# TheShadow29/VidSitu

Hardware: AMD Instinct MI355X
Metric: clips/s (10s@32x224x224) SlowFast+TxEnc fwd+bwd (higher is better)
Workload: dtype bf16

## Files before the change

### include/vidsitu_hip.h

```cpp
#ifndef VIDSITU_HIP_H
#define VIDSITU_HIP_H

#include <stddef.h>
#include <stdint.h>

#ifdef __cplusplus
extern "C" {
#endif

typedef enum vs_status {
  VS_OK = 0,
  VS_ERR_BAD_ARG = -1,
  VS_ERR_UNSUPPORTED = -2,
  VS_ERR_WORKSPACE = -3,
  VS_ERR_LAUNCH = -4
} vs_status;

#define VS_CONV_AFFINE 1
#define VS_CONV_RESIDUAL 2
#define VS_CONV_RELU 4
#define VS_CONV_STATS 8
#define VS_CONV_NAIVE 16
#define VS_CONV_TILE(id) (((id) + 1) << 8)
#define VS_CONV_RING(ns) (((ns) & 7) << 16)
// ... 40 lines not shown
int vs_stem_conv_wgrad(const void* dy, const void* x4, float* dwp, int N, int T, int H, int W,
                       int Cout, int kT, int dy_ld, void* workspace, size_t ws_bytes, void* stream);

int vs_conv_fwd(const void* x, const void* w, void* y, const vs_conv_desc* d, const float* scale,
                const float* shift, const void* residual, float* stats_partial,
                void* workspace, size_t ws_bytes, void* stream);
int vs_conv_stats_rows(const vs_conv_desc* d);
size_t vs_conv_workspace_bytes(const vs_conv_desc* d, int dgrad);
int vs_conv_plan(const vs_conv_desc* d, int dgrad, int* out);
int vs_conv_fwd_bc_fusable(const vs_conv_desc* d, int cout_c);
int vs_conv_fwd_bc(const void* x, const void* w_b, const vs_conv_desc* d, const float* scale_b,
                   const float* shift_b, const void* w_c, int cout_c, const float* scale_c,
                   const float* shift_c, const void* residual, int res_ld, void* y, int y_ld, int relu_c,
                   void* stream);

int vs_conv_dgrad(const void* dy, const void* wt, void* dx, const vs_conv_desc* d,
                  const void* residual, void* workspace, size_t ws_bytes, void* stream);

int vs_conv_dgrad_bnstats_rows(const vs_conv_desc* d);
int vs_conv_dgrad_bnstats(const void* dy, const void* wt, void* dx, const vs_conv_desc* d, const void* residual,
                          const void* bn_y, int bn_y_ld, const uint8_t* relu_bits, const float* mean,
                          const float* invstd, const float* gamma, const float* beta, float* stats_partial,
                          void* workspace, size_t ws_bytes, void* stream);

typedef struct vs_dgrad_epilogue {
  const void* residual;
  const uint8_t* residual_bits;
  const void* bn_y;
  int bn_y_ld;
  const uint8_t* relu_bits;
  const float* mean;
  const float* invstd;
  const float* gamma;
  const float* beta;
  float* stats_partial;
  const void* bn_y2;
  int bn_y2_ld;
  const float* mean2;
  const float* invstd2;
  float* stats_partial2;
} vs_dgrad_epilogue;
int vs_conv_dgrad_ex(const void* dy, const void* wt, void* dx, const vs_conv_desc* d,
                     const vs_dgrad_epilogue* ep, void* workspace, size_t ws_bytes, void* stream);
int vs_weight_transpose(const void* w, void* wt, int Cout, int taps, int Cin, void* stream);
int vs_weight_transpose_batched(const void* src, void* dst, const int64_t* table, int n,
                                int64_t total, void* stream);
int vs_transpose_f32_batched(const float* src, float* dst, const int64_t* table, int n, int64_t total,
                             void* stream);
int vs_weight_transpose_tiled(const void* src, void* dst, const int64_t* table, const int64_t* tile_first,
                              int n, int64_t total_tiles, int elem_bytes, void* stream);

#define VS_WGRAD_NODEEP (1 << 12)
#define VS_WGRAD_FORCEDEEP (1 << 13)
size_t vs_conv_wgrad_workspace_bytes(const vs_conv_desc* d);
int vs_conv_wgrad(const void* dy, const void* x, float* dw, const vs_conv_desc* d,
                  void* workspace, size_t ws_bytes, void* stream);
typedef struct vs_wgrad_item {
  const void* dy;
  const void* x;
  float* dw;
  vs_conv_desc d;
} vs_wgrad_item;
int vs_conv_wgrad_group_ok(const vs_wgrad_item* items, int n);
size_t vs_conv_wgrad_group_workspace_bytes(const vs_wgrad_item* items, int n);
int vs_conv_wgrad_group(const vs_wgrad_item* items, int n, void* workspace, size_t ws_bytes, void* stream);
int vs_conv_wgrad_partial(const void* dy, const void* x, float* dw, const vs_conv_desc* d, void* slabs,
                          size_t slab_bytes, int* splits, void* stream);
int64_t vs_wgrad_reduce_blocks(int64_t elements);
int vs_wgrad_reduce(const float* slabs, float* dw, int64_t elements, int splits, void* stream);
int vs_wgrad_reduce_batched(const int64_t* table, int n_entries, int64_t total_blocks, void* stream);
int vs_wgrad_reduce_defer(int mode);
int vs_wgrad_reduce_flush(void);

int vs_bn_finalize(const float* partials, int nparts, double count, const float* gamma,
                   const float* beta, float* running_mean, float* running_var, float momentum,
                   float eps, float* scale, float* shift, float* mean, float* invstd, int C,
                   void* stream);
size_t vs_bn_finalize_workspace_bytes(void);
int vs_bn_finalize_ws(const float* partials, int nparts, double count, const float* gamma, const float* beta,
                      float* running_mean, float* running_var, float momentum, float eps, float* scale,
                      float* shift, float* mean, float* invstd, int C, void* workspace, size_t ws_bytes,
                      void* stream);
int vs_bn_partials_reduce(const float* partials, int nparts, float* out, int C, int G,
                          void* stream);
int vs_bn_apply(const void* y, const float* scale, const float* shift, const void* residual,
                void* out, int64_t rows, int C, int y_ld, int res_ld, int out_ld, int relu,
                void* stream);
int vs_bn_apply_mask(const void* y, const float* scale, const float* shift, const void* residual,
                     void* out, uint8_t* relu_bits, int64_t rows, int C, int y_ld, int res_ld,
                     int out_ld, void* stream);
int vs_bn_apply2(const void* y, const float* scale, const float* shift, const void* y2, const float* scale2,
                 const float* shift2, void* out, uint8_t* relu_bits, int64_t rows, int C, int y_ld, int y2_ld,
                 int out_ld, void* stream);
int vs_bn_bwd_reduce(const void* dz, const void* z, const void* y, const float* mean,
                     const float* invstd, const float* gamma, const float* beta, float* partial,
                     int64_t rows, int C, int dz_ld, int z_ld, int y_ld, int relu, void* stream);
int vs_bn_bwd_reduce_rows(int64_t rows, int C);
int vs_bn_bwd_finalize(const float* partial, int nparts, float* dgamma, float* dbeta, int C,
                       void* stream);
int vs_bn_bwd_finalize_ws(const float* partial, int nparts, float* dgamma, float* dbeta, int C, void* workspace,
                          size_t ws_bytes, void* stream);
int vs_bn_bwd_apply(const void* dz, const void* z, const void* y, const float* mean,
                    const float* invstd, const float* gamma, const float* beta,
                    const float* dgamma, const float* dbeta, void* dy, void* dres, int64_t rows,
                    int C, int dz_ld, int z_ld, int y_ld, int dy_ld, int dres_ld, int relu,
                    void* stream);
// ... 211 lines not shown
```

### vidsitu_amd/_lib.py

```python
import ctypes as C
import os
import subprocess

_HERE = os.path.dirname(os.path.abspath(__file__))
LIB_PATH = os.environ.get("VS_LIB_PATH") or os.path.join(_HERE, "libvidsitu_hip.so")
CSRC_DIR = os.path.join(_HERE, "csrc")

VS_CONV_AFFINE = 1
VS_CONV_RESIDUAL = 2
VS_CONV_RELU = 4
VS_CONV_STATS = 8
VS_CONV_NAIVE = 16
VS_CONV_SPLITK = 1 << 15
VS_CONV_NOCLASS = 1 << 19
VS_CONV_NOHALO = 1 << 21
VS_CONV_FORCEHALO = 1 << 22
VS_CONV_NOPW = 1 << 23
VS_CONV_FORCEPW = 1 << 24
VS_CONV_DIRECTBNB = 1 << 25
VS_CONV_BNB2 = 1 << 26
VS_CONV_NODEEP = 1 << 27
VS_CONV_FORCEDEEP = 1 << 28
VS_CONV_SPLITK_IL = 1 << 29
VS_CONV_NOSPLITK_IL = 1 << 30
VS_WGRAD_NODEEP = 1 << 12
VS_WGRAD_FORCEDEEP = 1 << 13


def VS_CONV_TILE(tile_id):
    return (tile_id + 1) << 8


def VS_CONV_RING(stages):
    return (stages & 7) << 16


class ConvDesc(C.Structure):

    _fields_ = [
        (n, C.c_int32)
        for n in (
            "N Ti Hi Wi Cin To Ho Wo Cout kT kH kW sT sH sW pT pH pW x_ld y_ld res_ld flags"
        ).split()
    ]


class DgradEpilogue(C.Structure):

    _fields_ = [("residual", C.c_void_p), ("residual_bits", C.c_void_p), ("bn_y", C.c_void_p),
                ("bn_y_ld", C.c_int32), ("relu_bits", C.c_void_p), ("mean", C.c_void_p),
                ("invstd", C.c_void_p), ("gamma", C.c_void_p), ("beta", C.c_void_p),
                ("stats_partial", C.c_void_p), ("bn_y2", C.c_void_p), ("bn_y2_ld", C.c_int32),
                ("mean2", C.c_void_p), ("invstd2", C.c_void_p), ("stats_partial2", C.c_void_p)]


class WgradItem(C.Structure):

    _fields_ = [("dy", C.c_void_p), ("x", C.c_void_p), ("dw", C.c_void_p), ("d", ConvDesc)]


_p, _i, _i64, _f, _d, _sz = C.c_void_p, C.c_int, C.c_int64, C.c_float, C.c_double, C.c_size_t
_u32, _u64 = C.c_uint32, C.c_uint64
_dp = C.POINTER(ConvDesc)

SIGNATURES = {
    "vs_last_error_string": (C.c_char_p, []),
    "vs_version": (_i, []),
    "vs_launch_count": (_i64, []),
    "vs_pack_input": (_i, [_p, _i, _p, _i, _i, _i, _i, _i, _i, _p]),
    "vs_frames_u8_pack": (_i, [_p, _p, _p, _i, _i, _i, _i, _i, _i, _p, _p, _i, _p]),
    "vs_stem_conv_fwd": (_i, [_p, _p, _p, _i, _i, _i, _i, _i, _i, _i, _i, _p, _p, _p, _p]),
    "vs_stem_stats_rows": (_i, [_i, _i, _i, _i]),
    "vs_stem_wgrad_workspace_bytes": (_sz, [_i, _i, _i, _i, _i, _i]),
    "vs_stem_conv_wgrad": (_i, [_p, _p, _p, _i, _i, _i, _i, _i, _i, _i, _p, _sz, _p]),
    "vs_conv_fwd": (_i, [_p, _p, _p, _dp, _p, _p, _p, _p, _p, _sz, _p]),
    "vs_conv_stats_rows": (_i, [_dp]),
    "vs_conv_workspace_bytes": (_sz, [_dp, _i]),
    "vs_conv_plan": (_i, [_dp, _i, _p]),
    "vs_conv_fwd_bc_fusable": (_i, [_dp, _i]),
# ... 185 lines not shown
```

### vidsitu_amd/csrc/conv_wgrad.hip

```cpp
#include <stdlib.h>

#include "common.h"

#include <mutex>
#include <type_traits>
#include "glue_bodies.h"

typedef __attribute__((ext_vector_type(4))) short s16x4;
typedef __attribute__((address_space(3))) s16x4 lds_s16x4;

struct WgradP {
  const uint16_t* dy;
  const uint16_t* x;
  float* out;
  int P;
  int Cout, Kp, Cin, x_ld, dy_ld;
  int To, Ho, Wo, Ti, Hi, Wi;
  int kT, kH, kW, sT, sH, sW, pT, pH, pW;
  int tilesM, tilesN, S, rows_per_split;
  unsigned x_bytes, dy_bytes;
  int xcd_order;
  int dbg;
};

#define WG_OOB 0x80000000u

#define WG_ROWTAB 1024

__device__ __forceinline__ int wg_swz_chunk(int row) {
  return ((row & 3) << 1) | (((row >> 3) & 1) << 3);
}

#ifndef WG_NARROW_DEPTH
#define WG_NARROW_DEPTH 3
#endif
constexpr int wg_depth(int bm) { return bm <= 32 ? WG_NARROW_DEPTH : 2; }

template <int BM, int BN, int WM, int WN, int MODE>
__global__ __launch_bounds__(256) void conv_wgrad_kernel(WgradP p) {
  extern __shared__ __attribute__((aligned(16))) char smem[];
  constexpr int D = wg_depth(BM), R = D - 1;
  static_assert(D >= 2 && R * 64 < WG_ROWTAB / 2, "loads never run past the table half being rebuilt");
  constexpr int TM = BM / WM, TN = BN / WN;
  constexpr int MR = TM / 16, NR = TN / 16;
  constexpr int CM = BM / 8, CN = BN / 8;
  constexpr int RPM = 256 / CM, RPN = 256 / CN;
  constexpr int IM = (64 + RPM - 1) / RPM, IN = (64 + RPN - 1) / RPN;
  constexpr int IMG = 64 * 256;
  constexpr int STAGE = 2 * IMG;
  static_assert(WM * WN == 4, "4 waves");

  const int tid = threadIdx.x;
  int bid = blockIdx.x;
  if (p.xcd_order) {
    const int nwg = gridDim.x, q = nwg >> 3, r = nwg & 7, xcd = blockIdx.x & 7;
    bid = (xcd < r ? xcd * (q + 1) : r * (q + 1) + (xcd - r) * q) + (blockIdx.x >> 3);
  }
  const int ntile = p.tilesM * p.tilesN;
  const int s = bid / ntile;
// ... 843 lines not shown
      for (int u = 0; u < 8; ++u) v[u] = *(const float4*)(slabs + (long long)(s + u) * n + i * 4);
#pragma unroll
      for (int u = 0; u < 8; ++u) {
        acc.x += v[u].x;
        acc.y += v[u].y;
        acc.z += v[u].z;
        acc.w += v[u].w;
      }
    }
    for (; s < s1; ++s) {
      const float4 v = *(const float4*)(slabs + (long long)s * n + i * 4);
      acc.x += v.x;
      acc.y += v.y;
      acc.z += v.z;
      acc.w += v.w;
    }
  }
  part[sl][col] = acc;
  __syncthreads();
  if (sl == 0 && i < n4) {
    float4 t = part[0][col];
    for (int k = 1; k < 16; ++k) {
      const float4 v = part[k][col];
      t.x += v.x;
      t.y += v.y;
      t.z += v.z;
      t.w += v.w;
    }
    *(float4*)(dw + i * 4) = t;
  }
}

extern "C" int vs_wgrad_reduce_batched(const int64_t* table, int n_entries, int64_t total_blocks, void* stream) {
  VS_CHECK_ARG(table && n_entries > 0 && total_blocks > 0, "bad args");
  hipLaunchKernelGGL(wgrad_reduce_batched_kernel, dim3((unsigned)total_blocks), dim3(256), 0, (hipStream_t)stream,
                     (const long long*)table, n_entries);
  VS_CHECK_LAUNCH();
  return VS_OK;
}

extern "C" int64_t vs_wgrad_reduce_blocks(int64_t n) { return (n / 4 + 15) / 16; }

extern "C" int vs_wgrad_reduce(const float* slabs, float* dw, int64_t n, int splits, void* stream) {
  VS_CHECK_ARG(slabs && dw && n > 0 && splits > 1, "bad args");
  hipLaunchKernelGGL(wgrad_reduce_kernel, dim3((unsigned)wgrad_reduce_vblocks(n, splits)), dim3(256), 0, (hipStream_t)stream,
                     slabs, dw, (long long)n, splits);
  VS_CHECK_LAUNCH();
  return VS_OK;
}

struct WgCfg {
  int bm, bn, S, rows_per_split, tilesM, tilesN;
  int deep;
};


static bool wg_deep_plan(const vs_conv_desc* d, WgCfg* c) {
  static const int mode = [] { const char* e = getenv("VS_WGRAD_DEEP"); return e ? atoi(e) : 1; }();
  const bool force = mode == 2 || (d->flags & VS_WGRAD_FORCEDEEP);
  if (mode == 0 || (d->flags & VS_WGRAD_NODEEP)) return false;
  if (((d->flags >> 8) & 0xf) || ((d->flags >> 16) & 7) || ((d->flags >> 24) & 0xff)) return false;
  const int taps = d->kT * d->kH * d->kW;
  const int Kp = taps * d->Cin;
  const long long P = (long long)d->N * d->To * d->Ho * d->Wo;
  if (taps > 31 || Kp % 8 != 0 || d->Cout % 8 != 0) return false;
  const int tilesM = (d->Cout + 127) / 128, tilesN = (Kp + 255) / 256;
  const long long tiles = (long long)tilesM * tilesN;
  const double row_eff = (double)d->Cout / (128.0 * tilesM), col_eff = (double)Kp / (256.0 * tilesN);
  long long S = 256 / tiles;
  const long long maxS = P / 512;
  if (S > maxS) S = maxS;
  const long long slab_cap = (64ll << 20) / ((long long)d->Cout * Kp * 4);
  if (S > slab_cap) S = slab_cap;
  if (S < 1) S = 1;
  long long rps = (P + S - 1) / S;
  rps = (rps + 31) / 32 * 32;
  S = (P + rps - 1) / rps;
  if (!force && (row_eff < 0.9 || col_eff < 0.75 || tiles * S < 128 || tiles > 256 || rps < 512)) return false;
  static const long long min_p = [] { const char* e = getenv("VS_WGRAD_DEEP_MINP"); return e ? atoll(e) : 3000ll; }();
  if (!force && P < min_p) return false;
  if (tiles * S > 65535) return false;
  c->bm = 128;
  c->bn = 256;
  c->tilesM = tilesM;
  c->tilesN = tilesN;
  c->S = (int)S;
  c->rows_per_split = (int)rps;
  c->deep = 1;
  return true;
}

static const int kWgTiles[8][2] = {{128, 128}, {128, 64}, {64, 128}, {64, 64}, {32, 128}, {32, 64}, {16, 128}, {16, 64}};

static WgCfg wg_pick(const vs_conv_desc* d) {
  WgCfg c;
  c.deep = 0;
  if (wg_deep_plan(d, &c)) return c;
  const int Kp = d->kT * d->kH * d->kW * d->Cin;
  const long long P = (long long)d->N * d->To * d->Ho * d->Wo;
  c.bm = d->Cout >= 128 ? 128 : (d->Cout >= 64 ? 64 : (d->Cout >= 32 ? 32 : 16));
  c.bn = Kp >= 128 ? 128 : 64;
  if (d->Cout <= 16) c.bn = Kp > 64 ? 128 : 64;
  else if (d->Cout <= 32) c.bn = 64;
  const int forced = (d->flags >> 8) & 0xf;
  if (forced >= 1 && forced <= 8) {
    c.bm = kWgTiles[forced - 1][0];
    c.bn = kWgTiles[forced - 1][1];
  }
  c.tilesM = (d->Cout + c.bm - 1) / c.bm;
  c.tilesN = (Kp + c.bn - 1) / c.bn;
  const long long tiles = (long long)c.tilesM * c.tilesN;
  static const long long slots = [] {
    const char* e = getenv("VS_WGRAD_SLOTS");
    return e ? atoll(e) : 384ll;
  }();
  static const long long small_slots = [] {
    const char* e = getenv("VS_WGRAD_SLOTS_SMALL");
    return e ? atoll(e) : 512ll;
  }();
  long long target = (d->Cout <= 32) ? small_slots : slots;
  const int forced_slots = (d->flags >> 24) & 0xff;
  if (forced_slots) target = 8ll * forced_slots;
  long long S = target / tiles;
  static const long long s1_tiles = [] {
    const char* e = getenv("VS_WGRAD_S1_TILES");
    return e ? atoll(e) : 128ll;
  }();
  if (s1_tiles > 0 && tiles >= s1_tiles && !forced_slots) S = 1;
  const long long maxS = (P + 511) / 512;
  if (S > maxS) S = maxS;
  const long long slab_cap = (64ll << 20) / ((long long)d->Cout * Kp * 4);
  if (S > slab_cap) S = slab_cap;
  if (S > 1024) S = 1024;
  if (S < 1) S = 1;
  long long rps = (P + S - 1) / S;
  rps = (rps + 63) / 64 * 64;
  S = (P + rps - 1) / rps;
  c.S = (int)S;
  c.rows_per_split = (int)rps;
  return c;
}

extern "C" size_t vs_conv_wgrad_workspace_bytes(const vs_conv_desc* d) {
  const WgCfg c = wg_pick(d);
  if (c.S <= 1) return 0;
  return (size_t)c.S * d->Cout * d->kT * d->kH * d->kW * d->Cin * sizeof(float);
}

static bool pair_take_wgrad(const WgradP& p, int grid, size_t smem, int mode, hipStream_t st);
// ... 270 lines not shown
        while (t0 < nt) {
          const long long chunk = pos >> 5;
          const int room = 32 - (int)(pos & 31), c = nt - t0 < room ? nt - t0 : room;
          const int x = (int)(chunk & 7), slot0 = (int)(chunk >> 3) * 32 + (int)(pos & 31);
          if (cnt[x] == WGG_JOBS || slot0 + c > 510) { fits = false; break; }
          g.jobtab[x][cnt[x]++] = ((unsigned)slot0 << 23) | ((unsigned)a << 18) | ((unsigned)sp << 12) | (unsigned)t0;
          t0 += c;
          pos += c;
        }
      }
    }
    if (fits) {
      const long long chunks = (pos + 31) >> 5;
      int mx = 0;
      for (int x = 0; x < 8; ++x) {
        long long sl = 0;
        for (long long c = x; c < chunks; c += 8) sl = (c >> 3) * 32 + ((c == chunks - 1 && (pos & 31)) ? (pos & 31) : 32);
        g.jobend[x] = (unsigned short)sl;
        if ((int)sl > mx) mx = (int)sl;
      }
#ifdef VS_WGG_DEBUG
      for (int x = 0; x < 8; ++x) {
        fprintf(stderr, "xcd %d (%d slots):", x, (int)g.jobend[x]);
        for (int i = 0; i < cnt[x]; ++i) fprintf(stderr, " [slot %u p %u s %u t %u]", g.jobtab[x][i] >> 23, (g.jobtab[x][i] >> 18) & 31, (g.jobtab[x][i] >> 12) & 63, g.jobtab[x][i] & 4095);
        fprintf(stderr, "\n");
      }
      for (int a = 0; a < n; ++a) fprintf(stderr, "problem %d: tiles %d x %d S %d rps %d count %d\n", a, g.p[a].tilesM, g.p[a].tilesN, g.p[a].S, g.p[a].rows_per_split, g.count[a]);
#endif
      g.jobs = 1;
      grid = 8 * mx;
    }
  }
  static std::once_flag gattr;
  std::call_once(gattr, [] {
    (void)hipFuncSetAttribute((const void*)conv_wgrad_deep_group_kernel, hipFuncAttributeMaxDynamicSharedMemorySize, 160 * 1024);
  });
  const size_t smem = (size_t)WGD_NU * WGD_UNIT + 2 * WGD_TAB * sizeof(int2);
  hipLaunchKernelGGL(conv_wgrad_deep_group_kernel, dim3(grid), dim3(512), smem, (hipStream_t)stream, g);
  VS_CHECK_LAUNCH();
  if (r.n > 0) {
    hipLaunchKernelGGL(wgrad_reduce_group_kernel, dim3((unsigned)r.first[r.n]), dim3(256), 0, (hipStream_t)stream, r);
    VS_CHECK_LAUNCH();
  }
  return VS_OK;
}

static int wgrad_impl(const void* dy, const void* x, float* dw, const vs_conv_desc* d, void* workspace,
                      size_t ws_bytes, void* stream, bool reduce_now, int* splits_out) {
  VS_CHECK_ARG(d && dy && x && dw, "null argument");
  VS_CHECK_ARG(d->Cin % 8 == 0 && d->Cout % 8 == 0, "Cin and Cout must be multiples of 8");
  VS_CHECK_ARG(d->x_ld % 8 == 0 && d->y_ld % 8 == 0, "row pitches must be multiples of 8");
  VS_CHECK_ARG((long long)d->N * d->Ti * d->Hi * d->Wi < (1ll << 31), "too many positions");
  const WgCfg c = wg_pick(d);
  const size_t need = vs_conv_wgrad_workspace_bytes(d);
  if (need > 0 && (workspace == nullptr || ws_bytes < need)) {
    vs_set_error("vs_conv_wgrad: workspace too small (%zu < %zu)", ws_bytes, need);
    return VS_ERR_WORKSPACE;
  }
  if (g_pending.have && ((const void*)g_pending.r.slabs == workspace || g_pending.r.dw == dw)) pending_flush();
  WgradP p;
  {
    const int rc = wg_fill_params(p, dy, x, c.S > 1 ? (float*)workspace : dw, d, c);
    if (rc) return rc;
  }
  {
    static const int xo = [] { const char* e = getenv("VS_WGRAD_XCD"); return e ? atoi(e) : 1; }();
    p.xcd_order = xo && (c.tilesM * c.tilesN <= 32 || xo == 2 || (c.S % 8 == 0 && c.tilesM * c.tilesN <= 64));
    static const int dbg = [] { const char* e = getenv("VS_WGRAD_DBG"); return e ? atoi(e) : 0; }();
    p.dbg = dbg;
  }
  p.rows_per_split = c.rows_per_split;
  const bool dense = (d->kT * d->kH * d->kW == 1) && d->sT == 1 && d->sH == 1 && d->sW == 1 &&
                     d->pT == 0 && d->pH == 0 && d->pW == 0;
  const int mode = dense ? 0 : 1;
  hipStream_t st = (hipStream_t)stream;
  const int fring = (d->flags >> 16) & 7;
  int ring = fring == 1 ? 0 : (fring >= 2 ? (fring > 3 ? 3 : fring) : (c.bm == 128 ? 2 : 0));
  if (d->kT * d->kH * d->kW > 31) ring = 0;
  int rc;
  if (c.deep) {
    static std::once_flag dattr;
    std::call_once(dattr, [] {
      (void)hipFuncSetAttribute((const void*)conv_wgrad_deep_kernel<0, false>, hipFuncAttributeMaxDynamicSharedMemorySize, 160 * 1024);
      (void)hipFuncSetAttribute((const void*)conv_wgrad_deep_kernel<1, false>, hipFuncAttributeMaxDynamicSharedMemorySize, 160 * 1024);
      (void)hipFuncSetAttribute((const void*)conv_wgrad_deep_kernel<0, true>, hipFuncAttributeMaxDynamicSharedMemorySize, 160 * 1024);
      (void)hipFuncSetAttribute((const void*)conv_wgrad_deep_kernel<1, true>, hipFuncAttributeMaxDynamicSharedMemorySize, 160 * 1024);
    });
    static const int stag = [] { const char* e = getenv("VS_WGRAD_DEEP_STAG"); return e ? atoi(e) : 1; }();
    const size_t smem = (size_t)WGD_NU * WGD_UNIT + 2 * WGD_TAB * sizeof(int2);
    const int grid = p.tilesM * p.tilesN * p.S;
    if (stag && mode == 0) hipLaunchKernelGGL((conv_wgrad_deep_kernel<0, true>), dim3(grid), dim3(512), smem, st, p);
    else if (stag) hipLaunchKernelGGL((conv_wgrad_deep_kernel<1, true>), dim3(grid), dim3(512), smem, st, p);
    else if (mode == 0) hipLaunchKernelGGL((conv_wgrad_deep_kernel<0, false>), dim3(grid), dim3(512), smem, st, p);
    else hipLaunchKernelGGL((conv_wgrad_deep_kernel<1, false>), dim3(grid), dim3(512), smem, st, p);
    VS_CHECK_LAUNCH();
    rc = VS_OK;
  } else if (c.bm == 128 && c.bn == 128) rc = wg_launch<128, 128, 2, 2>(p, mode, ring, st);
  else if (c.bm == 128) rc = wg_launch<128, 64, 2, 2>(p, mode, ring, st);
  else if (c.bm == 64 && c.bn == 128) rc = wg_launch<64, 128, 2, 2>(p, mode, ring, st);
  else if (c.bm == 64) rc = wg_launch<64, 64, 2, 2>(p, mode, ring, st);
  else if (c.bm == 32 && c.bn == 128) rc = wg_launch<32, 128, 1, 4>(p, mode, ring, st);
  else if (c.bm == 32) rc = wg_launch<32, 64, 1, 4>(p, mode, ring, st);
  else if (c.bn == 128) rc = wg_launch<16, 128, 1, 4>(p, mode, ring, st);
  else rc = wg_launch<16, 64, 1, 4>(p, mode, ring, st);
  if (rc) return rc;
  if (splits_out) *splits_out = c.S;
  if (c.S > 1 && reduce_now) {
    const long long n = (long long)d->Cout * p.Kp;
    const long long grid = wgrad_reduce_vblocks(n, c.S);
    if (!pair_defer_reduce((const float*)workspace, dw, n, c.S) &&
        !pending_stash((const float*)workspace, dw, n, c.S, st)) {
      hipLaunchKernelGGL(wgrad_reduce_kernel, dim3((unsigned)grid), dim3(256), 0, st,
                         (const float*)workspace, dw, n, c.S);
      VS_CHECK_LAUNCH();
    }
  }
  return VS_OK;
}

extern "C" int vs_conv_wgrad(const void* dy, const void* x, float* dw, const vs_conv_desc* d,
                             void* workspace,
                             size_t ws_bytes, void* stream) {
  return wgrad_impl(dy, x, dw, d, workspace, ws_bytes, stream, true, nullptr);
}

extern "C" int vs_conv_wgrad_partial(const void* dy, const void* x, float* dw, const vs_conv_desc* d, void* slabs,
                                     size_t slab_bytes, int* splits, void* stream) {
  VS_CHECK_ARG(splits != nullptr, "null splits");
  return wgrad_impl(dy, x, dw, d, slabs, slab_bytes, stream, false, splits);
}
```

### vidsitu_amd/ops.py

```python
import ctypes as C

import torch

from . import _lib
from ._lib import (
    VS_CONV_AFFINE,
    VS_CONV_BNB2,
    VS_CONV_DIRECTBNB,
    VS_CONV_FORCEDEEP,
    VS_CONV_FORCEHALO,
    VS_CONV_FORCEPW,
    VS_CONV_NAIVE,
    VS_CONV_NOCLASS,
    VS_CONV_NODEEP,
    VS_CONV_NOHALO,
    VS_CONV_NOPW,
    VS_CONV_NOSPLITK_IL,
    VS_CONV_RELU,
    VS_CONV_RESIDUAL,
    VS_CONV_RING,
    VS_CONV_SPLITK,
    VS_CONV_SPLITK_IL,
    VS_CONV_STATS,
    VS_CONV_TILE,
    VS_WGRAD_FORCEDEEP,
    VS_WGRAD_NODEEP,
    ConvDesc,
)

BF16 = torch.bfloat16


def _stream():
    return C.c_void_p(torch.cuda.current_stream().cuda_stream)


def _ptr(t):
    if t is None:
        return None
    if not t.is_cuda:
        raise _lib.VsError("HIP op called with a non-GPU tensor (no CPU fallback exists)")
    return C.c_void_p(t.data_ptr())


def new_act(n, c, t, h, w, device, ctot=None, c_off=0, dtype=BF16, zero=False):
    ctot = c if ctot is None else ctot
    alloc = torch.zeros if zero else torch.empty
    buf = alloc((n, t, h, w, ctot), dtype=dtype, device=device)
    return buf.permute(0, 4, 1, 2, 3)[:, c_off : c_off + c]


def channel_slice(x, c_off, c):
    return x[:, c_off : c_off + c]


def act_ld(x):
    n, c, t, h, w = x.shape
    s = x.stride()
    ld = s[4] if w > 1 else (s[3] if h > 1 else (s[2] if t > 1 else s[0]))
    ok = (c == 1 or s[1] == 1) and ld >= c
    ok = ok and (w == 1 or s[4] == ld) and (h == 1 or s[3] == w * ld)
    ok = ok and (t == 1 or s[2] == h * w * ld) and (n == 1 or s[0] == t * h * w * ld)
    if not ok or x.dtype != BF16:
        raise _lib.VsError(f"not a bf16 channels-last activation: shape {tuple(x.shape)} stride {s}")
    if ld % 8 or (x.storage_offset() % 8):
        raise _lib.VsError("activation pitch / channel offset must be multiples of 8")
    return ld


def act_rows(x):
    n, c, t, h, w = x.shape
    return n * t * h * w


def pack_input(x, cpad=8):
    x = x.contiguous()
    n, c, t, h, w = x.shape
    y = new_act(n, cpad, t, h, w, x.device)
    _lib.call(
# ... 354 lines not shown
        return out

    def flush(self):
        if not self.pending:
            return
        sig = tuple(self.pending)
        ent = self.tables.get(sig)
        if ent is None:
            rows, first = [], 0
            lib = _lib.load()
            for slab_ptr, dw_ptr, n, S in self.pending:
                rows.append([slab_ptr, dw_ptr, n, S, first])
                first += int(lib.vs_wgrad_reduce_blocks(n))
            dev = torch.device("cuda", torch.cuda.current_device())
            ent = self.tables[sig] = (torch.tensor(rows, dtype=torch.int64, device=dev), len(rows), first)
        table, n_ent, blocks = ent
        _lib.call("vs_wgrad_reduce_batched", _ptr(table), n_ent, blocks, _stream())
        self.pending = []


WG_TILES = [(128, 128), (128, 64), (64, 128), (64, 64), (32, 128), (32, 64), (16, 128), (16, 64)]


WGRAD_GROUP_MAX = 20


def _wgrad_items(items):
    arr = (_lib.WgradItem * len(items))()
    for i, (dy, x, k, s, p, out) in enumerate(items):
        if not out.permute(0, 2, 3, 4, 1).is_contiguous() or out.dtype != torch.float32:
            raise _lib.VsError("conv_wgrad out must be fp32 with [Cout][taps][Cin] memory")
        arr[i].dy, arr[i].x, arr[i].dw = dy.data_ptr(), x.data_ptr(), out.data_ptr()
        arr[i].d = make_desc(x.shape, act_ld(x), dy.shape, act_ld(dy), k, s, p, 0)
        _ptr(dy), _ptr(x), _ptr(out)
    return arr


def conv_wgrad_group_ok(items):
    if not 1 <= len(items) <= WGRAD_GROUP_MAX:
        return False
    return bool(_lib.load().vs_conv_wgrad_group_ok(_wgrad_items(items), len(items)))


def conv_wgrad_group(items):
    if _WHATIF_WGRAD:
        return
    arr = _wgrad_items(items)
    need = int(_lib.load().vs_conv_wgrad_group_workspace_bytes(arr, len(items)))
    ws = _workspace(need, items[0][0].device, "wgrad") if need else None
    _lib.call("vs_conv_wgrad_group", arr, len(items), _ptr(ws), C.c_size_t(ws.numel() if ws is not None else 0),
              _stream())


def conv_wgrad(dy, x, k, s, p, out=None, ring=0, batch=None, tile=None, slots=0, deep=True):
    cout, cin = dy.shape[1], x.shape[1]
    if out is None:
        out = torch.empty((cout, *k, cin), dtype=torch.float32, device=x.device).permute(0, 4, 1, 2, 3)
    elif not out.permute(0, 2, 3, 4, 1).is_contiguous() or out.dtype != torch.float32:
        raise _lib.VsError("conv_wgrad out must be fp32 with [Cout][taps][Cin] memory")
    if batch is not None:
        return batch.wgrad(dy, x, k, s, p, out, ring)
    if _WHATIF_WGRAD:
        return out
    flags = ((ring & 7) << 16) | (((tile + 1) << 8) if tile is not None else 0) | (((slots // 8) & 0xff) << 24)
    if not deep:
        flags |= VS_WGRAD_NODEEP
    elif deep == "force":
        flags |= VS_WGRAD_FORCEDEEP
    d = make_desc(x.shape, act_ld(x), dy.shape, act_ld(dy), k, s, p, flags)
    need = _lib.load().vs_conv_wgrad_workspace_bytes(C.byref(d))
    ws = _workspace(need, x.device, "wgrad") if need else None
    _lib.call("vs_conv_wgrad", _ptr(dy), _ptr(x), _ptr(out), C.byref(d), _ptr(ws),
              C.c_size_t(ws.numel() if ws is not None else 0), _stream())
    return out


import os as _os
_WHATIF = int(_os.environ.get("VS_WHATIF", "0"))
_BN_TWO_LEVEL = int(_os.environ.get("VS_BN_TWO_LEVEL", "512"))
BN_FIN2 = _os.environ.get("VS_BN_FIN2", "1") != "0"
_fin_ws = [0]
_whatif_const = {}


def _fin_ws_bytes():
    if not _fin_ws[0]:
        _fin_ws[0] = int(_lib.load().vs_bn_finalize_workspace_bytes())
    return _fin_ws[0]



def bn_finalize(partials, count, gamma, beta, running_mean, running_var, momentum, eps, train):
    c = gamma.numel()
    dev = gamma.device
    scale = torch.empty(c, dtype=torch.float32, device=dev)
    shift = torch.empty(c, dtype=torch.float32, device=dev)
    mean = torch.empty(c, dtype=torch.float32, device=dev)
    invstd = torch.empty(c, dtype=torch.float32, device=dev)
    nparts = partials.shape[0] if train else 0
    if train and _WHATIF & 1:
        k = (c, str(dev))
        if k not in _whatif_const:
            _whatif_const[k] = (torch.ones(c, device=dev), torch.zeros(c, device=dev), torch.zeros(c, device=dev),
                                torch.ones(c, device=dev))
        return _whatif_const[k]
    if train and BN_FIN2:
        ws = _workspace(_fin_ws_bytes(), dev, "fin")
        _lib.call("vs_bn_finalize_ws", _ptr(partials), nparts, float(count), _ptr(gamma), _ptr(beta),
                  _ptr(running_mean), _ptr(running_var), float(momentum), float(eps), _ptr(scale), _ptr(shift),
                  _ptr(mean), _ptr(invstd), c, _ptr(ws), C.c_size_t(ws.numel()), _stream())
        return scale, shift, mean, invstd
    if train and nparts > _BN_TWO_LEVEL:
        lvl1 = torch.empty((32, 2, c), dtype=torch.float32, device=dev)
        _lib.call("vs_bn_partials_reduce", _ptr(partials), nparts, _ptr(lvl1), c, 32, _stream())
        partials, nparts = lvl1, 32
    _lib.call("vs_bn_finalize", _ptr(partials) if train else None, nparts, float(count),
              _ptr(gamma), _ptr(beta), _ptr(running_mean), _ptr(running_var), float(momentum),
              float(eps), _ptr(scale), _ptr(shift), _ptr(mean), _ptr(invstd), c, _stream())
    return scale, shift, mean, invstd


# ... 956 lines not shown
```

Measured before the change: 742.5.

## Add patch-tiled wgrad kernel for small-channel 1x3x3 convolutions

Adds a dedicated weight-gradient kernel for stride-1, padding-1 1x3x3 convolutions with up to 64 channels. Each block DMAs spatial patches of x, with halo, and of dy into LDS through a 2- or 3-deep buffer ring. It builds all nine taps from the shared patch using transposed LDS reads and MFMA, and writes per-split slabs that the existing reduction sums. By default it is used only for the 8→8 and 64→64 shapes of the SlowFast bottlenecks, and only when there are enough positions. The goal is to stop re-reading im2col-style data for each tap. The cost is extra plan and launch complexity and a workspace size that is now computed from the patch plan.

```diff
diff --git a/include/vidsitu_hip.h b/include/vidsitu_hip.h
--- a/include/vidsitu_hip.h
+++ b/include/vidsitu_hip.h
@@ -116,6 +116,8 @@
 
 #define VS_WGRAD_NODEEP (1 << 12)
 #define VS_WGRAD_FORCEDEEP (1 << 13)
+#define VS_WGRAD_NOPATCH (1 << 14)
+#define VS_WGRAD_PATCH (1 << 20)
 size_t vs_conv_wgrad_workspace_bytes(const vs_conv_desc* d);
 int vs_conv_wgrad(const void* dy, const void* x, float* dw, const vs_conv_desc* d,
                   void* workspace, size_t ws_bytes, void* stream);
diff --git a/vidsitu_amd/_lib.py b/vidsitu_amd/_lib.py
--- a/vidsitu_amd/_lib.py
+++ b/vidsitu_amd/_lib.py
@@ -25,6 +25,8 @@
 VS_CONV_NOSPLITK_IL = 1 << 30
 VS_WGRAD_NODEEP = 1 << 12
 VS_WGRAD_FORCEDEEP = 1 << 13
+VS_WGRAD_NOPATCH = 1 << 14
+VS_WGRAD_PATCH = 1 << 20
 
 
 def VS_CONV_TILE(tile_id):
diff --git a/vidsitu_amd/csrc/conv_wgrad.hip b/vidsitu_amd/csrc/conv_wgrad.hip
--- a/vidsitu_amd/csrc/conv_wgrad.hip
+++ b/vidsitu_amd/csrc/conv_wgrad.hip
@@ -5,6 +5,7 @@
 #include <mutex>
 #include <type_traits>
 #include "glue_bodies.h"
+#include "conv_wgrad_patch.h"
 
 typedef __attribute__((ext_vector_type(4))) short s16x4;
 typedef __attribute__((address_space(3))) s16x4 lds_s16x4;
@@ -954,6 +955,8 @@
 struct WgCfg {
   int bm, bn, S, rows_per_split, tilesM, tilesN;
   int deep;
+  int patch;
+  WgPatchPlan pp;
 };
 
 
@@ -994,9 +997,35 @@
 
 static const int kWgTiles[8][2] = {{128, 128}, {128, 64}, {64, 128}, {64, 64}, {32, 128}, {32, 64}, {16, 128}, {16, 64}};
 
+static bool wg_patch_default(const vs_conv_desc* d) {
+  const long long P = (long long)d->N * d->To * d->Ho * d->Wo;
+  const bool shape = (d->Cin == 8 && d->Cout == 8) || (d->Cin == 64 && d->Cout == 64);
+  return shape && P * 4 >= (long long)d->Cout * 9 * d->Cin * 16;
+}
+
+static bool wg_patch_plan(const vs_conv_desc* d, WgCfg* c) {
+  if (d->flags & VS_WGRAD_NOPATCH) return false;
+  const bool force = (d->flags & VS_WGRAD_PATCH) != 0;
+  if (!force && (((d->flags >> 8) & 0xf) || ((d->flags >> 16) & 7) || (d->flags & VS_WGRAD_FORCEDEEP))) return false;
+  const int forced_slots = (d->flags >> 24) & 0xff;
+  const long long target = forced_slots ? 8ll * forced_slots : (d->Cout <= 32 ? 512ll : 384ll);
+  if (!wgpatch_plan(d, target, &c->pp)) return false;
+  if (!force && !wg_patch_default(d)) return false;
+  c->patch = 1;
+  c->deep = 0;
+  c->bm = 64;
+  c->bn = 128;
+  c->tilesM = c->tilesN = 1;
+  c->S = c->pp.S;
+  c->rows_per_split = c->pp.ips;
+  return true;
+}
+
 static WgCfg wg_pick(const vs_conv_desc* d) {
   WgCfg c;
   c.deep = 0;
+  c.patch = 0;
+  if (wg_patch_plan(d, &c)) return c;
   if (wg_deep_plan(d, &c)) return c;
   const int Kp = d->kT * d->kH * d->kW * d->Cin;
   const long long P = (long long)d->N * d->To * d->Ho * d->Wo;
@@ -1373,7 +1402,7 @@
   VS_CHECK_ARG(d->x_ld % 8 == 0 && d->y_ld % 8 == 0, "row pitches must be multiples of 8");
   VS_CHECK_ARG((long long)d->N * d->Ti * d->Hi * d->Wi < (1ll << 31), "too many positions");
   const WgCfg c = wg_pick(d);
-  const size_t need = vs_conv_wgrad_workspace_bytes(d);
+  const size_t need = c.S > 1 ? (size_t)c.S * d->Cout * d->kT * d->kH * d->kW * d->Cin * sizeof(float) : 0;
   if (need > 0 && (workspace == nullptr || ws_bytes < need)) {
     vs_set_error("vs_conv_wgrad: workspace too small (%zu < %zu)", ws_bytes, need);
     return VS_ERR_WORKSPACE;
@@ -1399,7 +1428,9 @@
   int ring = fring == 1 ? 0 : (fring >= 2 ? (fring > 3 ? 3 : fring) : (c.bm == 128 ? 2 : 0));
   if (d->kT * d->kH * d->kW > 31) ring = 0;
   int rc;
-  if (c.deep) {
+  if (c.patch) {
+    rc = wgpatch_launch(dy, x, c.S > 1 ? (float*)workspace : dw, d, c.pp, st);
+  } else if (c.deep) {
     static std::once_flag dattr;
     std::call_once(dattr, [] {
       (void)hipFuncSetAttribute((const void*)conv_wgrad_deep_kernel<0, false>, hipFuncAttributeMaxDynamicSharedMemorySize, 160 * 1024);
diff --git a/vidsitu_amd/csrc/conv_wgrad_patch.h b/vidsitu_amd/csrc/conv_wgrad_patch.h
--- /dev/null
+++ b/vidsitu_amd/csrc/conv_wgrad_patch.h
@@ -0,0 +1,18 @@
+#pragma once
+#include "common.h"
+
+struct WgPatchPlan {
+  int mr, ntw, wn;
+  int TH;
+  int tilesH, tilesW;
+  int nitems;
+  int S, ips;
+  int lcx;
+  int nb;
+  size_t smem;
+};
+
+bool wgpatch_plan(const vs_conv_desc* d, long long target, WgPatchPlan* pl);
+
+int wgpatch_launch(const void* dy, const void* x, float* out, const vs_conv_desc* d, const WgPatchPlan& pl,
+                   hipStream_t st);
diff --git a/vidsitu_amd/csrc/conv_wgrad_patch.hip b/vidsitu_amd/csrc/conv_wgrad_patch.hip
--- /dev/null
+++ b/vidsitu_amd/csrc/conv_wgrad_patch.hip
@@ -0,0 +1,360 @@
+#include "conv_wgrad_patch.h"
+
+#include <mutex>
+
+typedef __attribute__((ext_vector_type(4))) short wp_s16x4;
+typedef __attribute__((address_space(3))) wp_s16x4 wp_lds_s16x4;
+typedef __attribute__((ext_vector_type(8))) short wp_s16x8;
+
+#define WGP_OOB 0x80000000u
+#define WGP_PW 18
+
+struct WgPatchP {
+  const uint16_t* dy;
+  const uint16_t* x;
+  float* out;
+  int Cout, Cin, Kp, x_ld, dy_ld;
+  int H, W;
+  int TH, tilesH, tilesW, nitems, ips;
+  int lcx, nb;
+  unsigned x_bytes, dy_bytes;
+};
+
+__device__ __forceinline__ bf16x8 wp_tr_pair(const char* p0, const char* p1) {
+  const wp_s16x4 lo = __builtin_amdgcn_ds_read_tr16_b64_v4i16((wp_lds_s16x4*)p0);
+  const wp_s16x4 hi = __builtin_amdgcn_ds_read_tr16_b64_v4i16((wp_lds_s16x4*)p1);
+  return __builtin_bit_cast(bf16x8, (wp_s16x8)__builtin_shufflevector(lo, hi, 0, 1, 2, 3, 4, 5, 6, 7));
+}
+
+__device__ __forceinline__ int wp_xchunk(int c, int pcol, int lcx) {
+  if (lcx == 3) return c ^ ((((pcol >> 1) & 1) | (((pcol >> 3) & 1) << 1)) << 1);
+  if (lcx == 2) return c ^ (((pcol >> 3) & 1) << 1);
+  return c;
+}
+
+template <int MR>
+__device__ __forceinline__ int wp_yoff(int k, int c) {
+  if (MR == 4) return k * 128 + ((c ^ ((((k >> 1) & 1) | (((k >> 3) & 1) << 1)) << 1)) << 4);
+  if (MR == 2) return k * 64 + ((c ^ (((k >> 3) & 1) << 1)) << 4);
+  return ((k ^ (((k >> 3) & 1) << 2)) << 5) + (c << 4);
+}
+
+template <int MR, int NTW, int WN, int NL>
+__global__ __launch_bounds__(256) void conv_wgrad_patch_kernel(WgPatchP p) {
+  extern __shared__ __attribute__((aligned(16))) char smem[];
+  constexpr int WK = 4 / WN;
+  static_assert(WN == 1 || WN == 2 || WN == 4, "waves across the columns");
+  const int tid = threadIdx.x, lane = tid & 63;
+  const int wave = __builtin_amdgcn_readfirstlane(tid >> 6);
+  const int wn = wave % WN, wk = wave / WN;
+  const int g = lane >> 4, li = lane & 15, q = li >> 2, p4 = li & 3;
+
+  const int RX = 16 << p.lcx;
+  constexpr int YC = 2 * MR;
+  const int npp = (p.TH + 2) * WGP_PW, npos = p.TH * 16;
+  const int nx = npp << p.lcx, ny = npos * YC;
+  const int nlx = (nx + 255) >> 8, nly = (ny + 255) >> 8;
+  const int YIMG = nlx * 4096;
+  const int BUF = (nlx + nly) * 4096;
+  const int cxm = (1 << p.lcx) - 1;
+  const int ncx = p.Cin >> 3, ncy = p.Cout >> 3;
+  const unsigned xpitch = (unsigned)(p.x_ld * 2), dypitch = (unsigned)(p.dy_ld * 2);
+  const int nks = p.TH >> 1;
+
+  int meta[NL], goff[NL];
+#pragma unroll
+  for (int i = 0; i < NL; ++i) {
+    meta[i] = 0;
+    goff[i] = 0;
+    if (i < nlx) {
+      const int id = tid + 256 * i;
+      const int pp = id >> p.lcx;
+      const int prow = pp / WGP_PW, pcol = pp - prow * WGP_PW;
+      const int c = wp_xchunk(id & cxm, pcol, p.lcx);
+      if (id < nx && c < ncx) {
+        meta[i] = prow | (pcol << 6) | (1 << 11);
+        goff[i] = ((prow - 1) * p.W + (pcol - 1)) * (int)xpitch + c * 16;
+      }
+    } else if (i < nlx + nly) {
+      const int id = tid + 256 * (i - nlx);
+      int k, c;
+      if (MR == 4) {
+        k = id >> 3;
+        c = (id & 7) ^ ((((k >> 1) & 1) | (((k >> 3) & 1) << 1)) << 1);
+      } else if (MR == 2) {
+        k = id >> 2;
+        c = (id & 3) ^ (((k >> 3) & 1) << 1);
+      } else {
+        const int slot = id >> 1;
+        k = slot ^ (((slot >> 3) & 1) << 2);
+        c = id & 1;
+      }
+      if (id < ny && c < ncy) {
+        meta[i] = ((k >> 4) + 1) | (((k & 15) + 1) << 6) | (1 << 11);
+        goff[i] = ((k >> 4) * p.W + (k & 15)) * (int)dypitch + c * 16;
+      }
+    }
+  }
+
+  typedef __attribute__((address_space(3))) char* lds_ptr_t;
+  const unsigned lds0 = (unsigned)(unsigned long)(lds_ptr_t)smem + (unsigned)wave * 1024u;
+  auto rsrc_words = [](const void* base, unsigned bytes) __attribute__((always_inline)) {
+    const unsigned long a = (unsigned long)base;
+    return (i32x4){(int)(unsigned)a, (int)((unsigned)(a >> 32) & 0xffffu), (int)bytes, 0x00020000};
+  };
+  const i32x4 xdesc = rsrc_words(p.x, p.x_bytes), dydesc = rsrc_words(p.dy, p.dy_bytes);
+  auto dma16 = [](const i32x4& desc, unsigned lds_addr, unsigned voff) __attribute__((always_inline)) {
+    asm volatile("s_mov_b32 m0, %0\n\ts_nop 0\n\tbuffer_load_dwordx4 %1, %2, 0 offen lds"
+                 :
+                 : "s"(lds_addr), "v"(voff), "s"(desc)
+                 : "memory");
+  };
+  auto dma = [&](int item, int buf) __attribute__((always_inline)) {
+    const int tw = item % p.tilesW, t1 = item / p.tilesW;
+    const int th = t1 % p.tilesH, f = t1 / p.tilesH;
+    const int h0 = th * p.TH, w0 = tw * 16;
+    const int pos0 = (f * p.H + h0) * p.W + w0;
+    const unsigned xbase = (unsigned)pos0 * xpitch, dybase = (unsigned)pos0 * dypitch;
+    const unsigned B = lds0 + (unsigned)(buf * BUF);
+#pragma unroll
+    for (int i = 0; i < NL; ++i) {
+      if (i < nlx + nly) {
+        int m = meta[i];
+        asm volatile("" : "+v"(m));
+        const int h = h0 + (m & 63) - 1, w = w0 + ((m >> 6) & 31) - 1;
+        const bool ok = (m >> 11) && (unsigned)h < (unsigned)p.H && (unsigned)w < (unsigned)p.W;
+        if (i < nlx) dma16(xdesc, B + i * 4096, ok ? xbase + (unsigned)goff[i] : WGP_OOB);
+        else dma16(dydesc, B + i * 4096, ok ? dybase + (unsigned)goff[i] : WGP_OOB);
+      }
+    }
+  };
+
+  const int clane = 8 * (g & 1) + q;
+  int boff_lo[NTW], boff_hi[NTW];
+#pragma unroll
+  for (int j = 0; j < NTW; ++j) {
+    int col = (j * WN + wn) * 16 + 4 * p4;
+    if (col >= p.Kp) col = 0;
+    const int tap = col / p.Cin, ci = col - tap * p.Cin;
+    const int dh = tap / 3, dw = tap - dh * 3;
+    const int pl = clane + dw, ph = pl + 4;
+    boff_lo[j] = (dh * WGP_PW + pl) * RX + (wp_xchunk(ci >> 3, pl, p.lcx) << 4) + (ci & 7) * 2;
+    boff_hi[j] = (dh * WGP_PW + ph) * RX + (wp_xchunk(ci >> 3, ph, p.lcx) << 4) + (ci & 7) * 2;
+  }
+
+  f32x4 acc[MR][NTW];
+#pragma unroll
+  for (int a = 0; a < MR; ++a)
+#pragma unroll
+    for (int j = 0; j < NTW; ++j) acc[a][j] = (f32x4){0.f, 0.f, 0.f, 0.f};
+
+  auto compute = [&](int buf) __attribute__((always_inline)) {
+    const char* X = smem + buf * BUF;
+    const char* Y = X + YIMG;
+    for (int ks = wk; ks < nks; ks += WK) {
+      const int k = ks * 32 + 8 * g + q;
+      bf16x8 af[MR];
+#pragma unroll
+      for (int a = 0; a < MR; ++a)
+        af[a] = wp_tr_pair(Y + wp_yoff<MR>(k, 2 * a) + p4 * 8, Y + wp_yoff<MR>(k + 4, 2 * a) + p4 * 8);
+      const char* xr = X + (ks * 2 + (g >> 1)) * (WGP_PW * RX);
+      constexpr int PD = MR == 4 ? 3 : (MR == 2 ? 4 : 6);
+      bf16x8 bq[PD];
+#pragma unroll
+      for (int j = 0; j < PD - 1; ++j)
+        if (j < NTW) bq[j] = wp_tr_pair(xr + boff_lo[j], xr + boff_hi[j]);
+#pragma unroll
+      for (int j = 0; j < NTW; ++j) {
+        if (j + PD - 1 < NTW) bq[(j + PD - 1) % PD] = wp_tr_pair(xr + boff_lo[j + PD - 1], xr + boff_hi[j + PD - 1]);
+#pragma unroll
+        for (int a = 0; a < MR; ++a) acc[a][j] = __builtin_amdgcn_mfma_f32_16x16x32_bf16(af[a], bq[j % PD], acc[a][j], 0, 0, 0);
+      }
+    }
+  };
+
+  const int np = nlx + nly, nb = p.nb;
+  auto wait_landed = [&](bool younger) __attribute__((always_inline)) {
+    if (!younger) { asm volatile("s_waitcnt vmcnt(0)" ::: "memory"); return; }
+    switch (np) {
+      case 1: asm volatile("s_waitcnt vmcnt(1)" ::: "memory"); break;
+      case 2: asm volatile("s_waitcnt vmcnt(2)" ::: "memory"); break;
+      case 3: asm volatile("s_waitcnt vmcnt(3)" ::: "memory"); break;
+      case 4: asm volatile("s_waitcnt vmcnt(4)" ::: "memory"); break;
+      case 5: asm volatile("s_waitcnt vmcnt(5)" ::: "memory"); break;
+      case 6: asm volatile("s_waitcnt vmcnt(6)" ::: "memory"); break;
+      default: asm volatile("s_waitcnt vmcnt(0)" ::: "memory"); break;
+    }
+  };
+  const int item0 = blockIdx.x * p.ips, item1 = min(p.nitems, item0 + p.ips);
+  for (int d = 0; d < nb - 1; ++d)
+    if (item0 + d < item1) dma(item0 + d, d);
+  int cur = 0, nxt = nb - 1;
+  for (int it = item0; it < item1; ++it) {
+    wait_landed(nb == 3 && it + 1 < item1);
+    __syncthreads();
+    if (it + nb - 1 < item1) dma(it + nb - 1, nxt);
+    __builtin_amdgcn_sched_barrier(0);
+    compute(cur);
+    __builtin_amdgcn_sched_barrier(0);
+    cur = cur + 1 == nb ? 0 : cur + 1;
+    nxt = nxt + 1 == nb ? 0 : nxt + 1;
+  }
+  __syncthreads();
+
+  if constexpr (WK > 1) {
+    float* R = (float*)smem;
+    for (int w = 1; w < WK; ++w) {
+      if (w > 1) __syncthreads();
+#pragma unroll
+      for (int a = 0; a < MR; ++a)
+#pragma unroll
+        for (int j = 0; j < NTW; ++j)
+#pragma unroll
+          for (int r = 0; r < 4; ++r) {
+            float* e = R + ((((wn * MR + a) * NTW + j) * 4 + r) << 6) + lane;
+            if (wk == w) *e = acc[a][j][r];
+          }
+      __syncthreads();
+      if (wk == 0) {
+#pragma unroll
+        for (int a = 0; a < MR; ++a)
+#pragma unroll
+          for (int j = 0; j < NTW; ++j)
+#pragma unroll
+            for (int r = 0; r < 4; ++r) acc[a][j][r] += R[((((wn * MR + a) * NTW + j) * 4 + r) << 6) + lane];
+      }
+    }
+  }
+  if (wk != 0) return;
+  float* dst = p.out + (long long)blockIdx.x * p.Cout * p.Kp;
+#pragma unroll
+  for (int a = 0; a < MR; ++a)
+#pragma unroll
+    for (int j = 0; j < NTW; ++j) {
+      const int col = (j * WN + wn) * 16 + li;
+#pragma unroll
+      for (int r = 0; r < 4; ++r) {
+        const int row = a * 16 + g * 4 + r;
+        if (row < p.Cout && col < p.Kp) dst[(long long)row * p.Kp + col] = acc[a][j][r];
+      }
+    }
+}
+
+#define WGP_NL 10
+#ifndef WGP_MAXPASS
+#define WGP_MAXPASS 6
+#endif
+#define WGP_LDS_MAX (80 * 1024)
+
+static int wgp_log2ceil(int v) {
+  int l = 0;
+  while ((1 << l) < v) ++l;
+  return l;
+}
+
+bool wgpatch_plan(const vs_conv_desc* d, long long target, WgPatchPlan* pl) {
+  if (d->kT != 1 || d->kH != 3 || d->kW != 3 || d->sT != 1 || d->sH != 1 || d->sW != 1 || d->pT != 0 || d->pH != 1 ||
+      d->pW != 1)
+    return false;
+  if (d->Cin % 8 || d->Cout % 8 || d->Cin < 8 || d->Cout < 8 || d->Cin > 64 || d->Cout > 64) return false;
+  if (d->x_ld % 8 || d->y_ld % 8 || d->x_ld < d->Cin || d->y_ld < d->Cout) return false;
+  if (d->To != d->Ti || d->Ho != d->Hi || d->Wo != d->Wi || d->N < 1 || d->Ti < 1 || d->Hi < 1 || d->Wi < 1) return false;
+  const long long frames = (long long)d->N * d->Ti;
+  const long long P = frames * d->Hi * d->Wi;
+  if (P * d->x_ld * 2 >= (1ll << 31) || P * d->y_ld * 2 >= (1ll << 31)) return false;
+  const int Kp = 9 * d->Cin, NT = (Kp + 15) / 16;
+  const int mr = d->Cout <= 16 ? 1 : (d->Cout <= 32 ? 2 : 4);
+  int ntw, wn;
+  if (NT <= 5) { ntw = 5; wn = 1; }
+  else if (NT <= 9) { ntw = 9; wn = 1; }
+  else if (NT <= 18) { ntw = mr == 1 ? 18 : 9; wn = mr == 1 ? 1 : 2; }
+  else { ntw = mr == 1 ? 18 : 9; wn = mr == 1 ? 2 : 4; }
+  const int lcx = wgp_log2ceil(d->Cin / 8);
+  const size_t red = 4 / wn > 1 ? (size_t)wn * mr * ntw * 1024 : 0;
+  auto passes = [&](int th) { return ((((th + 2) * WGP_PW) << lcx) + 255) / 256 + (th * 16 * 2 * mr + 255) / 256; };
+  auto buf_bytes = [&](int th) { return (size_t)passes(th) * 4096; };
+  if (target < 1) target = 1;
+  const int heven = (d->Hi + 1) / 2 * 2;
+  const int tilesW = (d->Wi + 15) / 16;
+  int TH = 0;
+  {
+    double best_eff = -1.0;
+    long long most = -1;
+    int th_most = 0;
+    for (int th = heven; th >= 2; th -= 2) {
+      if (passes(th) > WGP_MAXPASS || th > 60) continue;
+      const int tiles = (d->Hi + th - 1) / th;
+      const long long items = frames * tiles * tilesW;
+      if (items > most) { most = items; th_most = th; }
+      if (items < 3 * target) continue;
+      const double eff = (double)d->Hi / ((double)tiles * th);
+      if (eff > best_eff + 1e-9) { best_eff = eff; TH = th; }
+    }
+    if (TH == 0) TH = th_most;
+  }
+  if (TH == 0) return false;
+  const int tilesH = (d->Hi + TH - 1) / TH;
+  const long long nitems = frames * tilesH * tilesW;
+  if (nitems >= (1ll << 30)) return false;
+  long long S = target < nitems ? target : nitems;
+  const long long slab_cap = (64ll << 20) / ((long long)d->Cout * Kp * 4);
+  if (S > slab_cap) S = slab_cap;
+  if (S > 1024) S = 1024;
+  if (S < 1) S = 1;
+  const long long ips = (nitems + S - 1) / S;
+  S = (nitems + ips - 1) / ips;
+  pl->mr = mr; pl->ntw = ntw; pl->wn = wn;
+  pl->TH = TH; pl->tilesH = tilesH; pl->tilesW = tilesW;
+  pl->nitems = (int)nitems; pl->S = (int)S; pl->ips = (int)ips;
+  pl->lcx = lcx;
+  pl->nb = 3 * buf_bytes(TH) <= WGP_LDS_MAX ? 3 : 2;
+  const size_t bufs = pl->nb * buf_bytes(TH);
+  pl->smem = bufs > red ? bufs : red;
+  return pl->smem <= WGP_LDS_MAX;
+}
+
+template <int MR, int NTW, int WN>
+static int wgp_launch(const WgPatchP& p, const WgPatchPlan& pl, hipStream_t st) {
+  constexpr int NL = WGP_NL;
+  static std::once_flag attr;
+  std::call_once(attr, [] {
+    (void)hipFuncSetAttribute((const void*)conv_wgrad_patch_kernel<MR, NTW, WN, NL>,
+                              hipFuncAttributeMaxDynamicSharedMemorySize, WGP_LDS_MAX);
+  });
+  hipLaunchKernelGGL((conv_wgrad_patch_kernel<MR, NTW, WN, NL>), dim3(pl.S), dim3(256), pl.smem, st, p);
+  VS_CHECK_LAUNCH();
+  return VS_OK;
+}
+
+int wgpatch_launch(const void* dy, const void* x, float* out, const vs_conv_desc* d, const WgPatchPlan& pl,
+                   hipStream_t st) {
+  WgPatchP p;
+  p.dy = (const uint16_t*)dy;
+  p.x = (const uint16_t*)x;
+  p.out = out;
+  p.Cout = d->Cout; p.Cin = d->Cin; p.Kp = 9 * d->Cin;
+  p.x_ld = d->x_ld; p.dy_ld = d->y_ld;
+  p.H = d->Hi; p.W = d->Wi;
+  p.TH = pl.TH; p.tilesH = pl.tilesH; p.tilesW = pl.tilesW; p.nitems = pl.nitems; p.ips = pl.ips;
+  p.lcx = pl.lcx; p.nb = pl.nb;
+  const long long P = (long long)d->N * d->Ti * d->Hi * d->Wi;
+  p.x_bytes = (unsigned)(P * d->x_ld * 2);
+  p.dy_bytes = (unsigned)(P * d->y_ld * 2);
+#define WGP_CASE(MR_, NTW_, WN_) \
+  if (pl.mr == MR_ && pl.ntw == NTW_ && pl.wn == WN_) return wgp_launch<MR_, NTW_, WN_>(p, pl, st)
+  WGP_CASE(1, 5, 1);
+  WGP_CASE(1, 9, 1);
+  WGP_CASE(1, 18, 1);
+  WGP_CASE(1, 18, 2);
+  WGP_CASE(2, 5, 1);
+  WGP_CASE(2, 9, 1);
+  WGP_CASE(2, 9, 2);
+  WGP_CASE(2, 9, 4);
+  WGP_CASE(4, 5, 1);
+  WGP_CASE(4, 9, 1);
+  WGP_CASE(4, 9, 2);
+  WGP_CASE(4, 9, 4);
+#undef WGP_CASE
+  vs_set_error("vs_conv_wgrad: no patch kernel instance (%d, %d, %d)", pl.mr, pl.ntw, pl.wn);
+  return VS_ERR_UNSUPPORTED;
+}
diff --git a/vidsitu_amd/ops.py b/vidsitu_amd/ops.py
--- a/vidsitu_amd/ops.py
+++ b/vidsitu_amd/ops.py
@@ -25,6 +25,8 @@
     VS_CONV_TILE,
     VS_WGRAD_FORCEDEEP,
     VS_WGRAD_NODEEP,
+    VS_WGRAD_NOPATCH,
+    VS_WGRAD_PATCH,
     ConvDesc,
 )
 
@@ -485,7 +487,7 @@
               _stream())
 
 
-def conv_wgrad(dy, x, k, s, p, out=None, ring=0, batch=None, tile=None, slots=0, deep=True):
+def conv_wgrad(dy, x, k, s, p, out=None, ring=0, batch=None, tile=None, slots=0, deep=True, patch=None):
     cout, cin = dy.shape[1], x.shape[1]
     if out is None:
         out = torch.empty((cout, *k, cin), dtype=torch.float32, device=x.device).permute(0, 4, 1, 2, 3)
@@ -500,6 +502,8 @@
         flags |= VS_WGRAD_NODEEP
     elif deep == "force":
         flags |= VS_WGRAD_FORCEDEEP
+    if patch is not None:
+        flags |= VS_WGRAD_PATCH if patch else VS_WGRAD_NOPATCH
     d = make_desc(x.shape, act_ld(x), dy.shape, act_ld(dy), k, s, p, flags)
     need = _lib.load().vs_conv_wgrad_workspace_bytes(C.byref(d))
     ws = _workspace(need, x.device, "wgrad") if need else None
```

After: 741.0. About the same (-0.2%).
